# tnibler/local-features

Measured on AMD Instinct MI355X. Metric: MKD descriptors/sec (32x32 patch, 128-D), higher is better.
Workload: dtype f32 (f16x3 split MFMA pooling)

## Files before the change

local-features_amd/csrc/lf_mkd.cpp:

```cpp
#include "../../include/lf_mkd.h"

#include <hip/hip_runtime.h>

#include <algorithm>
#include <chrono>
#include <cmath>
#include <cstdlib>
#include <cstring>
#include <new>
#include <string>
#include <utility>
#include <vector>

#include "lf_mkd_internal.h"
#include "mkd_consts.hpp"
#include "mkd_device.h"

using namespace lfmkd;

namespace {

enum Memory { kDevice, kPinned };

template <typename T, Memory M = kDevice, bool Recorded = false>
// ... 107 lines not shown
struct DetectPlan {
    Recording graph;
    std::vector<uint32_t> cuts;
    std::vector<Recording> heads;
};

}

struct lf_mkd {
    lf_mkd_params params{};
    hipStream_t stream = nullptr;
    hipStream_t side_stream = nullptr;
    std::vector<hipEvent_t> side_events;
    struct {
        HipArray<short> colmap, colmap_unfolded;
        HipArray<float> pool_b_f32, white_a_f32, white_bias;
        HipArray<uint16_t> pool_b_f16, pool_b_fp6, white_a_f16, white_a_f16_unfolded;
    } consts;
    DeviceConsts dc;
    uint64_t batch = 0;
    HipArray<float> d_patches;
    HipArray<float> d_out;
    HipArray<float> d_kps;
    PyramidDesc pd{};
    HipArray<float> d_image, d_pyr, d_tmp_a, d_tmp_b;
    bool have_image = false;
    uint32_t max_frames = 1, n_frames = 0;
    long pyr_stride = 0;
    int n_layers = 7;
    HipArray<float> d_coarse;
    long layer_stride = 0, coarse_stride = 0;
// ... 158 lines not shown
        LF_CREATE_HIP(hipGetDeviceProperties(&prop, params->device));
        h->num_cus = prop.multiProcessorCount > 0 ? prop.multiProcessorCount : 256;
    }
    auto &c = h->consts;
    LF_CREATE_HIP(upload(c.colmap, hc.colmap));
    LF_CREATE_HIP(upload(c.pool_b_f32, hc.pool_b_f32));
    LF_CREATE_HIP(upload(c.pool_b_f16, hc.pool_b_f16));
    if (h->params.pool_mode == LF_MKD_POOL_F16_FP6) {
        LF_CREATE_HIP(upload(c.pool_b_fp6, hc.pool_b_fp6));
        LF_CREATE_HIP(upload(c.colmap_unfolded, hc.colmap_unfolded));
        LF_CREATE_HIP(upload(c.white_a_f16_unfolded, hc.white_a_f16_unfolded));
    }
    LF_CREATE_HIP(upload(c.white_a_f16, hc.white_a_f16));
    LF_CREATE_HIP(upload(c.white_a_f32, hc.white_a_f32));
    LF_CREATE_HIP(upload(c.white_bias, hc.white_bias));
    h->dc = DeviceConsts{c.colmap, c.pool_b_f32, c.pool_b_f16, c.white_a_f16, c.white_a_f32, c.colmap_unfolded, c.pool_b_fp6,
                         c.white_a_f16_unfolded, c.white_bias};
    LF_CREATE_HIP(h->d_totals.allocate(8));
    if (h->params.flags & LF_MKD_FLAG_KERNEL_TIMING) {
        LF_CREATE_HIP(h->d_clk.allocate(4));
        LF_CREATE_HIP(hipMemset(h->d_clk, 0, 4 * sizeof(unsigned long long)));
    }
    if (params->max_image_width && params->max_image_height) {
        if ((uint64_t(params->max_image_width) + 2 * kPyrApron) * (uint64_t(params->max_image_height) + 2 * kPyrApron) >= (1ull << 30) ||
            params->max_image_width >= (1u << 20) || params->max_image_height >= (1u << 20)) {
            h->err = "max_image_width x max_image_height (with the pyramid's apron of 48 texels a side) must stay below 2^30 pixels";
            return bail(LF_MKD_ERR_BAD_ARG);
        }
        h->max_frames = params->max_frames ? params->max_frames : 1;
        const size_t px = size_t(params->max_image_width) * params->max_image_height * h->max_frames;
        h->pyr_stride = pyramid_floats(params->max_image_width, params->max_image_height);
        h->layer_stride = long(params->max_image_width) * params->max_image_height;
// ... 334 lines not shown

int lfmkd_test_pool_tables(const float *mean, const float *eigvals, const float *eigvecs, float *pool_b_f32, int16_t *colmap, float *parity_defect) {
    if (!mean || !eigvals || !eigvecs) return LF_MKD_ERR_BAD_ARG;
    PcaModel pca;
    pca.mean.assign(mean, mean + kRaw);
    pca.eigvals.assign(eigvals, eigvals + kRaw);
    pca.eigvecs.assign(eigvecs, eigvecs + size_t(kRaw) * kRaw);
    HostConsts hc;
    if (const std::string e = build_host_consts(pca, hc); !e.empty()) {
        g_create_error = e;
        return LF_MKD_ERR_BAD_ARG;
    }
    if (pool_b_f32) std::memcpy(pool_b_f32, hc.pool_b_f32.data(), hc.pool_b_f32.size() * 4);
    if (colmap) std::memcpy(colmap, hc.colmap.data(), hc.colmap.size() * 2);
    if (parity_defect) *parity_defect = hc.lut_parity_defect;
    return LF_MKD_OK;
}

int lf_mkd_plan_upload(uint32_t width, uint32_t height, uint32_t bytes_per_pixel, uint32_t n_scales, uint32_t *cuts,
                       uint32_t max_cuts, uint32_t *n_cuts, double *modelled_us, double *one_piece_us) {
    if (!n_cuts || (bytes_per_pixel != 1 && bytes_per_pixel != 4) || width < 2 || height < 2 || (max_cuts && !cuts))
        return LF_MKD_ERR_BAD_ARG;
    const int n_layers = int(n_scales ? n_scales : 4) + 3;
    if (n_layers - 1 > 8) return LF_MKD_ERR_BAD_ARG;
    const std::vector<uint32_t> c = plan_cuts(n_layers, width, height, bytes_per_pixel == 1);
    *n_cuts = uint32_t(c.size());
    for (size_t i = 0; i < c.size() && i < max_cuts; ++i) cuts[i] = c[i];
    const FrontModel m;
    if (modelled_us) *modelled_us = front_finish_us(c, c.size() + 1, int(width), int(height), int(bytes_per_pixel), n_layers, m);
    if (one_piece_us) *one_piece_us = front_finish_us({}, 1, int(width), int(height), int(bytes_per_pixel), n_layers, m);
// ... 1154 lines not shown
```

local-features_amd/csrc/mkd_consts.cpp:

```cpp
#include "mkd_consts.hpp"

#include <cmath>
#include <cstdio>
#include <cstdlib>
#include <cstring>

namespace lfmkd {

namespace {

const float kVmN3K8[4] = {0.37872374f, 0.51796234f, 0.46882015f, 0.39798096f};
const float kVmN1K1[2] = {0.618176f, 0.6934725f};
const float kVmN2K8[3] = {0.37872374f, 0.51796234f, 0.46882015f};

struct Grid {
    float x[kPx], y[kPx];
    Grid() {
        for (int r = 0; r < kPatch; ++r)
            for (int c = 0; c < kPatch; ++c) {
                x[r * kPatch + c] = 2.f * float(c) / float(kPatch - 1) - 1.f;
                y[r * kPatch + c] = 2.f * float(r) / float(kPatch - 1) - 1.f;
            }
    }
};
// ... 248 lines not shown
        for (int y = 0; y < kPatch; ++y)
            for (int x = 0; x < kPatch / 2; ++x) {
                const double a = lut_value(col, y * kPatch + x), b = lut_value(col, y * kPatch + kPatch - 1 - x);
                even_err = std::fmax(even_err, std::fabs(a - b));
                odd_err = std::fmax(odd_err, std::fabs(a + b));
                mx = std::fmax(mx, std::fmax(std::fabs(a), std::fabs(b)));
            }
        defect = std::fmax(defect, float(std::fmin(even_err, odd_err) / mx));
        return memo = even_err <= odd_err ? 1 : -1;
    };
    FoldLayout fl;
    if (const std::string e = build_fold_layout(parity, fl); !e.empty()) return e;
    hc.lut_parity_defect = defect;
    if (!(defect < 1e-4f))
        return "internal: a pooling LUT column is neither even nor odd in x (defect " + std::to_string(defect) + ")";
    hc.colmap.assign(kPackedCols, -1);
    {
        std::vector<int> seen(kRaw, 0);
        for (int t = 0; t < kTiles; ++t) {
            int ut, v;
            acc_tile_source(t, ut, v);
            for (int c = 0; c < kTileCols; ++c) {
                const FoldColumn &fc = fl.col[ut][c];
                const int d = v ? fc.desc_v : fc.desc_u;
                if (d < 0) continue;
                hc.colmap[t * kTileCols + c] = int16_t(v && fc.sign_v < 0 ? -2 - d : d);
                ++seen[d];
            }
        }
        for (int d = 0; d < kRaw; ++d)
// ... 118 lines not shown
```

local-features_amd/csrc/mkd_consts.hpp:

```cpp
#pragma once
#include <cstdint>
#include <string>
#include <vector>

namespace lfmkd {

constexpr int kPatch = 32;
constexpr int kPx = kPatch * kPatch;
constexpr int kDimsIn = 7;
constexpr int kCart = 9;
constexpr int kPolar = 25;
constexpr int kRaw = 238;
constexpr int kOut = 128;

constexpr int kStreams = 7;
constexpr int kTiles = 21;
constexpr int kAccTiles = kTiles;
constexpr int kTileCols = 16;
constexpr int kPolarSlots = 10;
constexpr int kPackedCols = kTiles * kTileCols;
constexpr int kUniqueTiles = 12;

constexpr int kUnfAccTiles = 24;
constexpr int kUnfUniqueTiles = 15;
// ... 8 lines not shown
    std::vector<float> gradient_angle;
    std::vector<float> embedding_polar;
    std::vector<float> embedding_cartesian;
    std::vector<float> mean;
    std::vector<float> w_t;

    std::vector<int16_t> colmap;
    std::vector<float> pool_b_f32;
    std::vector<uint16_t> pool_b_f16;
    std::vector<uint16_t> white_a_f16;
    std::vector<float> white_a_f32;
    std::vector<int16_t> colmap_unfolded;
    std::vector<uint16_t> pool_b_fp6;
    std::vector<uint16_t> white_a_f16_unfolded;
    float lut_parity_defect = 0.f;
    std::vector<float> white_bias;
};

std::string build_host_consts(const PcaModel &pca, HostConsts &out);

}
```

local-features_amd/csrc/mkd_describe.hip:

```cpp
#include <hip/hip_runtime.h>
#include <stdint.h>

#include <type_traits>

#include "mkd_ablate.h"
#include "mkd_device.h"
#include "mkd_sample.h"

namespace lfmkd {


namespace {

typedef _Float16 f16x8 __attribute__((ext_vector_type(8)));
typedef unsigned int u32x4 __attribute__((ext_vector_type(4)));
typedef float f32x2 __attribute__((ext_vector_type(2)));
__device__ __forceinline__ f32x2 pk_fma(f32x2 a, f32x2 b, f32x2 c) { return __builtin_elementwise_fma(a, b, c); }
__device__ __forceinline__ f32x2 pk_set(float v) { return f32x2{v, v}; }

__device__ __host__ constexpr bool f16_family(int pool) { return pool == LF_POOL_F16X3 || pool == LF_POOL_F16_FP6; }

__device__ __host__ constexpr bool fold_form(int pool) { return pool != LF_POOL_F16_FP6; }
constexpr int kTiles = 21;
constexpr int kAccTiles = 21, kUnfAccTiles = 24;
__device__ __host__ constexpr int acc_tiles(bool fold) { return fold ? kAccTiles : kUnfAccTiles; }
__device__ __host__ constexpr int lut_pieces(bool fold) { return fold ? 24 : 30; }
constexpr int kPolarSlots = 10;

constexpr float kB0 = 0.0096f, kB1 = 0.2054f, kB2 = 0.5699f;

__device__ __host__ constexpr int row_bytes(bool fold) { return lut_pieces(fold) * 1024; }
__device__ __host__ constexpr int ring_off(bool fold) { return 2 * row_bytes(fold); }
constexpr int kRowBytes = row_bytes(true), kRingOff = ring_off(true);
constexpr int kRingSlots = 6;
[[maybe_unused]] constexpr int kSrcPatches = 0, kSrcKeypoints = 1, kSrcKeypointsSplit = 2;
constexpr int kRingSlotsKp = 12;
constexpr int kLevelTableBytes = 5 * kMaxPyrLevels * 4;

__device__ __forceinline__ float lane_fetch(int byte_addr, float v) {
    return __int_as_float(__builtin_amdgcn_ds_bpermute(byte_addr, __float_as_int(v)));
}

__device__ __forceinline__ void lds_dma16(const void *gsrc, void *ldst) {
    __builtin_amdgcn_global_load_lds((const __attribute__((address_space(1))) void *)gsrc,
                                     (__attribute__((address_space(3))) void *)ldst, 16, 0, 0);
}
__device__ __forceinline__ void lds_dma16_sv(const unsigned char *uniform_base, unsigned lane_off, void *ldst) {
    asm("" : "+s"(uniform_base));
    asm volatile("" : "+v"(lane_off));
    lds_dma16(uniform_base + lane_off, ldst);
}

template <int W, bool FOLD = true>
__device__ __forceinline__ void issue_lut_row(const unsigned char *__restrict__ lut_rows, int row,
                                              unsigned char *lds_row, int wave, int lane) {
    constexpr int kPieces = lut_pieces(FOLD);
    const unsigned lane16 = (unsigned)lane * 16u;
#pragma unroll
    for (int j = 0; j < (kPieces + W - 1) / W; ++j) {
        if (wave + W * j < kPieces) {
            const unsigned char *g = lut_rows + ((size_t)row * row_bytes(FOLD) + (size_t)(wave + W * j) * 1024);
            lds_dma16_sv(g, lane16, lds_row + (wave + W * j) * 1024);
        }
    }
}

constexpr int kWStepBytes = 16384;
__device__ __forceinline__ constexpr int wstage_slot(int step) { return step % 3 == 0 ? 0 : (step % 3 == 1 ? 32768 : 16384); }
static_assert(wstage_slot(0) + kWStepBytes <= row_bytes(true) && wstage_slot(10) >= row_bytes(false) &&
              wstage_slot(10) + kWStepBytes <= 2 * row_bytes(true), "both forms' row buffers");

template <int W>
__device__ __forceinline__ void issue_w_step(const unsigned char *__restrict__ wfrag, int step, unsigned char *lds,
                                             int wave, int lane) {
    const unsigned lane16 = (unsigned)lane * 16u;
    unsigned char *d = lds + wstage_slot(step);
#pragma unroll
// ... 340 lines not shown
    }
#pragma unroll
    for (int x = 0; x < 4; ++x) out[4 + x] = ob[3 - x];
    const float hal = lane_fetch(addr_l, out[3]), hbr = lane_fetch(addr_l, ob[0]);
    const float har = lane_fetch(addr_r, out[0]), hbl = lane_fetch(addr_r, ob[3]);
    nb[0] = has_l ? hal : out[0];
    nb[1] = has_r ? har : ob[0];
    nb[2] = has_r ? hbl : out[3];
    nb[3] = has_l ? hbr : ob[3];
}

__device__ __forceinline__ void fold_sum(const f32x2 (&s)[4], f32x2 &e0, f32x2 &e1) { e0 = s[0] + s[2]; e1 = s[1] + s[3]; }
__device__ __forceinline__ void fold_diff(const f32x2 (&s)[4], f32x2 &o0, f32x2 &o1) { o0 = s[0] - s[2]; o1 = s[1] - s[3]; }
__device__ __forceinline__ void fold_diff_rev(const f32x2 (&s)[4], f32x2 &o0, f32x2 &o1) { o0 = s[2] - s[0]; o1 = s[3] - s[1]; }

template <int POOL>
__device__ __forceinline__ void pool_harmonics(const f32x2 (&m)[4], const f32x2 (&c1)[4], const f32x2 (&s1)[4],
                                               const unsigned char *brow, BFrag &g, f32x4 (&acc)[kAccTiles]) {
    f32x2 pk[4], qk[4], pp[4], qp[4], tc[4];
    AFrag<POOL> au, av;
#pragma unroll
    for (int e = 0; e < 4; ++e) { pk[e] = m[e] * c1[e]; qk[e] = m[e] * s1[e]; tc[e] = c1[e] + c1[e]; }
#pragma unroll
    for (int k = 0; k < 3; ++k) {
        {
            f32x2 u[4], v[4];
            fold_sum(pk, u[0], u[1]);
            fold_diff(qk, u[2], u[3]);
            fold_sum(qk, v[0], v[1]);
            fold_diff_rev(pk, v[2], v[3]);
            if constexpr (POOL == LF_POOL_F16X3) {
                AFrag<POOL>::set2(au, u, av, v);
            } else {
                au.set(u);
                av.set(v);
            }
        }
        if (k < 2) {
#pragma unroll
            for (int e = 0; e < 4; ++e) {
                const f32x2 pn = pk_fma(tc[e], pk[e], k == 0 ? -m[e] : -pp[e]);
                const f32x2 qn = k == 0 ? tc[e] * qk[e] : pk_fma(tc[e], qk[e], -qp[e]);
                pp[e] = pk[e]; qp[e] = qk[e];
                pk[e] = pn; qk[e] = qn;
            }
        }
        const int a0 = 3 + 6 * k, u0 = 3 + 3 * k;
        const BFrag t0 = g, t1 = load_b(brow, u0 + 1), t2 = load_b(brow, u0 + 2);
        if (k < 2) g = load_b(brow, u0 + 3);
        mma_part<POOL, 0>(au, t0, acc[a0 + 0]); mma_part<POOL, 0>(av, t0, acc[a0 + 1]); mma_part<POOL, 0>(au, t1, acc[a0 + 2]);
        mma_part<POOL, 0>(av, t1, acc[a0 + 3]); mma_part<POOL, 0>(au, t2, acc[a0 + 4]); mma_part<POOL, 0>(av, t2, acc[a0 + 5]);
        mma_part<POOL, 1>(au, t0, acc[a0 + 0]); mma_part<POOL, 1>(av, t0, acc[a0 + 1]); mma_part<POOL, 1>(au, t1, acc[a0 + 2]);
        mma_part<POOL, 1>(av, t1, acc[a0 + 3]); mma_part<POOL, 1>(au, t2, acc[a0 + 4]); mma_part<POOL, 1>(av, t2, acc[a0 + 5]);
        mma_part<POOL, 2>(au, t0, acc[a0 + 0]); mma_part<POOL, 2>(av, t0, acc[a0 + 1]); mma_part<POOL, 2>(au, t1, acc[a0 + 2]);
        mma_part<POOL, 2>(av, t1, acc[a0 + 3]); mma_part<POOL, 2>(au, t2, acc[a0 + 4]); mma_part<POOL, 2>(av, t2, acc[a0 + 5]);
    }
}

typedef float v16f __attribute__((ext_vector_type(16)));
typedef unsigned v6u __attribute__((ext_vector_type(6)));
typedef int v8i __attribute__((ext_vector_type(8)));

__device__ __forceinline__ void pool_harmonics_fp6(const f32x2 (&m)[4], const f32x2 (&c1)[4], const f32x2 (&s1)[4],
// ... 188 lines not shown
#pragma unroll
            for (int rr = 0; rr < 4; ++rr)
                o[r0 + rr] = __builtin_amdgcn_mfma_f32_16x16x32_f16(__builtin_bit_cast(f16x8, src[2 * rr]), yl, o[r0 + rr], 0, 0, 0);
#pragma unroll
            for (int rr = 0; rr < 4; ++rr)
                o[r0 + rr] = __builtin_amdgcn_mfma_f32_16x16x32_f16(__builtin_bit_cast(f16x8, src[2 * rr]), yh, o[r0 + rr], 0, 0, 0);
        };
#pragma unroll
        for (int s = 0; s < 11; ++s) {
            if (s == 0) wait_vmcnt<2 * kDma>();
            else if (s < 10) wait_vmcnt<kDma>();
            else wait_vmcnt<0>();
            asm volatile("s_waitcnt lgkmcnt(0)" ::: "memory");
            __syncthreads();
            if (s >= 1 && s + 2 < 11) issue_w_step<W>(wfrag, s + 2, s_mem, wave, lane);
            if (s == 10 && more) issue_lut_row<W, kFold>(lut_rows, 0, s_mem, wave, lane);
            read_unit(2 * s, wbuf[0]);
            __builtin_amdgcn_sched_barrier(0);
            if (s > 0) mma_unit(2 * s - 1, wbuf[1]);
            {
                const f32x4 y0 = acc[2 * s];
                const f32x4 y1 = 2 * s + 1 < kTiles ? acc[(2 * s + 1 < kTiles) ? 2 * s + 1 : 0] : f32x4{0.f, 0.f, 0.f, 0.f};
                const f32x2 y[4] = {{y0[0], y0[1]}, {y0[2], y0[3]}, {y1[0], y1[1]}, {y1[2], y1[3]}};
                AFrag<LF_POOL_F16X3> yb;
                yb.set(y);
                yh = __builtin_bit_cast(f16x8, yb.hi);
                yl = __builtin_bit_cast(f16x8, yb.lo);
            }
            __builtin_amdgcn_sched_barrier(0);
            read_unit(2 * s + 1, wbuf[1]);
            __builtin_amdgcn_sched_barrier(0);
// ... 199 lines not shown
    sm.load_geometry(walk.cur, 0);
#pragma unroll 1
    for (int quarter = 0; quarter < 7; ++quarter) {
        sm.request(quarter, 0, ta);
        sm.finish(quarter, 0, 0, ta);
    }
    sm.request(7, 0, ta);
#pragma unroll 1
    for (long batch = walk.cur; batch < walk.end; batch += walk.step) {
        const bool more = batch + walk.step < walk.end;
        if (more) sm.load_geometry(batch + walk.step, set ^ 1);
        const int slot1 = (slot0 + 8) % kRingSlotsKp;
        auto step = [&](int g, KpTaps &cur, KpTaps &nxt) {
            asm volatile("s_waitcnt vmcnt(0) lgkmcnt(0)" ::: "memory");
            __syncthreads();
            if (g < 31) issue_lut_row<W>(lut_rows, g + 1, s_mem + ((g + 1) & 1) * kRowBytes, pw, lane);
            const int qn = g + 8;
            if (qn < 32) sm.request(qn, set, nxt);
            else if (more) sm.request(qn - 32, set ^ 1, nxt);
            __builtin_amdgcn_sched_barrier(0);
            const int qc = g + 7;
            if (qc < 32) sm.finish(qc, set, slot0, cur);
            else if (more) sm.finish(qc - 32, set ^ 1, slot1, cur);
        };
#pragma unroll 1
        for (int g = 0; g < ablate::kRows; g += 2) {
            step(g, ta, tb);
            step(g + 1, tb, ta);
        }
        asm volatile("s_waitcnt vmcnt(0) lgkmcnt(0)" ::: "memory");
#pragma unroll 1
// ... 29 lines not shown
    sm.load_geometry(batch, 0);
    sm.request(sp.q_first, 0, ta);
#pragma unroll 1
    for (int i = 0; i + 1 < sp.n_pro; i += 2) {
        sm.request(sp.q_first + i + 1, 0, tb);
        sm.finish(sp.q_first + i, 0, 0, ta);
        sm.request(sp.q_first + i + 2, 0, ta);
        sm.finish(sp.q_first + i + 1, 0, 0, tb);
    }
    sm.finish(sp.q_first + sp.n_pro - 1, 0, 0, ta);
    const int q_step0 = sp.q_first + sp.n_pro;
    if (q_step0 < sp.q_end) sm.request(q_step0, 0, ta);
    auto step = [&](int st, KpTaps &cur, KpTaps &nxt) {
        asm volatile("s_waitcnt vmcnt(0) lgkmcnt(0)" ::: "memory");
        __syncthreads();
        if (sp.lo + st + 1 < sp.hi) issue_lut_row<W>(lut_rows, sp.lo + st + 1, s_mem + ((st + 1) & 1) * kRowBytes, pw, lane);
        if (q_step0 + st + 1 < sp.q_end) sm.request(q_step0 + st + 1, 0, nxt);
        __builtin_amdgcn_sched_barrier(0);
        if (q_step0 + st < sp.q_end) sm.finish(q_step0 + st, 0, 0, cur);
    };
#pragma unroll 1
    for (int st = 0; st < sp.hi - sp.lo; st += 2) {
        step(st, ta, tb);
        step(st + 1, tb, ta);
    }
    asm volatile("s_waitcnt vmcnt(0) lgkmcnt(0)" ::: "memory");
    if (sp.consumer) {
#pragma unroll 1
        for (int e = 0; e < 12; ++e) __syncthreads();
    }
}

constexpr int kSplitSpinMax = 1 << 21;

}

template <int ANGLE, int POOL, int W, int SRC>
__global__ __launch_bounds__(SRC != kSrcPatches ? 128 * W : 64 * W) void mkd_pool(
    const float *__restrict__ patches, long n_host, const unsigned long long *__restrict__ n_dev,
    const unsigned char *__restrict__ lut_rows, const short *__restrict__ colmap, const unsigned char *__restrict__ wfrag,
    const float *__restrict__ bias, float *__restrict__ out, float *__restrict__ raw_out,
    std::conditional_t<SRC != kSrcPatches, KpSource, int> ks, unsigned long long *__restrict__ clk) {
    constexpr bool kKp = SRC != kSrcPatches, kSplit = SRC == kSrcKeypointsSplit;
    static_assert(!kSplit || W == 2, "the row-split form is the narrow (2 + 2 wave) form");
    if (clk && blockIdx.x == 0 && threadIdx.x == 0) {
        clk[0] = __builtin_readcyclecounter();
        clk[1] = __builtin_amdgcn_s_memrealtime();
    }
    constexpr int kSlots = kKp ? kRingSlotsKp : kRingSlots;
    static_assert(!kKp || POOL == LF_POOL_F16X3, "keypoint mode pools in f16x3");
    constexpr int kMPool = POOL == LF_POOL_F16_FP6 ? LF_POOL_F16X3 : POOL;
    constexpr bool kFold = fold_form(POOL);
    static_assert(!kKp || kFold, "the producers write the folded forms' LDS map");
    constexpr int kNAcc = acc_tiles(kFold), kRowB = row_bytes(kFold), kRingO = ring_off(kFold);
    __shared__ __attribute__((aligned(16))) unsigned char s_mem[kRingO + W * kSlots * 2048 +
                                                                (kKp ? kLevelTableBytes + kMaxPyrLevels * 8 : 0)];
    const long n = n_dev ? (long)*n_dev : n_host;
    const int lane = threadIdx.x & 63;
    const int wave = __builtin_amdgcn_readfirstlane(threadIdx.x >> 6);
    const int p = lane & 15, q = lane >> 4;
    const int addr_l = ((lane - 16) & 63) * 4, addr_r = ((lane + 16) & 63) * 4;
    const bool has_l = q > 0, has_r = q < 3;
    const long nbatch = (n + 16 * W - 1) / (16 * W);
    unsigned char *ring = s_mem + kRingO + wave * (kSlots * 2048);
    BatchWalk walk{(long)blockIdx.x, nbatch, (long)gridDim.x};
    [[maybe_unused]] RowSpan span{0, 32, 0, 32, 7, true};
    [[maybe_unused]] int role = 0, n_roles = 1;
    if constexpr (kKp) {
// ... 23 lines not shown
        __syncthreads();
        const LevelTable lt{ks.pd.levels, lv, lv + kMaxPyrLevels, lv + 2 * kMaxPyrLevels, lv + 3 * kMaxPyrLevels};
        if (wave >= W) {
            if constexpr (kSplit) kp_produce_split<W>(ks, lt, lv_off, n, walk.cur, span, s_mem, lut_rows, wave - W, lane);
            else kp_produce<W>(ks, lt, lv_off, n, walk, s_mem, lut_rows, wave - W, lane);
            return;
        }

        if constexpr (ablate::kConsumerPrio >= 0) __builtin_amdgcn_s_setprio(ablate::kConsumerPrio);
    }
    const unsigned char *ring_lane = kFold ? ring + (q * 16 + p) * 16 : ring + (q >> 1) * 1024 + ((2 * (q & 1)) * 16 + p) * 16;
    [[maybe_unused]] const unsigned char *ring_mirror = ring + 1024 + ((3 - q) * 16 + p) * 16;

    long batch = walk.cur;
    if (batch >= walk.end) return;
    auto raw_src = [&](const float *pt, long b) {
        const long b0 = b * (16 * W) + wave * 16;
        const long wave0 = b0 < n ? b0 : n - 1;
        const long pidx = b0 + p < n ? b0 + p : n - 1;
        return RawSrc{reinterpret_cast<const unsigned char *>(pt + wave0 * 1024), (unsigned)(pidx - wave0) * 4096u + 16u * q};
    };
    {
        if constexpr (!kKp) {
            const RawSrc src = raw_src(patches, batch);
#pragma unroll
            for (int r = -2; r <= 3; ++r) issue_raw_row(src, r, ring, r + 2);
        }
        issue_lut_row<W, kFold>(lut_rows, kSplit ? span.lo : 0, s_mem, wave, lane);
    }
    int slot0 = 0;
    unsigned par = 0;
    ablate::PhaseClock phase;
    phase.start();

    for (; batch < walk.end; batch += walk.step) {
        const unsigned char *wf = wfrag, *lr = lut_rows;
        const float *bs = bias, *pt = patches;
        float *o = out, *ro = raw_out;
        const short *cm = colmap;
        asm volatile("" : "+s"(wf), "+s"(bs), "+s"(lr), "+s"(o), "+s"(ro), "+s"(cm), "+s"(pt));
        const long base = batch * (16 * W) + wave * 16;
        const bool more = batch + walk.step < walk.end;
        const RawSrc src = kKp ? RawSrc{nullptr, 0u} : raw_src(pt, batch);
        const RawSrc src_next = !kKp && more ? raw_src(pt, batch + walk.step) : src;

        f32x4 acc[kNAcc];
#pragma unroll
        for (int t = 0; t < kNAcc; ++t) acc[t] = f32x4{0.f, 0.f, 0.f, 0.f};
        float cur[8], prv[8], cur_nb[4] = {0.f, 0.f, 0.f, 0.f};
        int s0 = 1;

        auto patch_row = [&](auto kind, const int g) __attribute__((always_inline)) {
            constexpr bool kFirst = decltype(kind)::value == 0, kLast = decltype(kind)::value == 2;
            constexpr bool kFirstInner = decltype(kind)::value == 3;

            phase.mark(7);
            if constexpr (!ablate::kNoRowSync) {
                asm volatile("s_waitcnt vmcnt(0)" ::: "memory");
                __syncthreads();
            }
            phase.mark(0);
            const unsigned char *brow = s_mem + par * kRowB + lane * 16;
            if (f16_family(POOL) ? !kLast : (!kLast || more)) {
                if constexpr (!kKp) issue_lut_row<W, kFold>(lr, (g + 1) & 31, s_mem + (par ^ 1) * kRowB, wave, lane);
            } else if (f16_family(POOL)) {
                issue_w_step<W>(wf, 0, s_mem, wave, lane);
            }
            par ^= 1;
            BFrag bm[3] = {load_b(brow, 0), load_b(brow, 1), load_b(brow, 2)};

            if constexpr (!kKp)
                if (!kFirst && !kLast && g <= 29) issue_raw_row(src, g + 4, ring, s0 == 0 ? kRingSlots - 1 : s0 - 1);
            auto kp_slot = [&](int y, int i) {
                int r_ = y - 2 + i;
                r_ = r_ < 0 ? 0 : (r_ > 31 ? 31 : r_);
                return (slot0 + r_) % kRingSlotsKp;
            };
            auto blur = [&](auto tap, float (&o)[8], float (&o_nb)[4]) __attribute__((always_inline)) {
                if constexpr (kFold) blur_row_fold_impl(ring_lane, ring_mirror, tap, addr_l, addr_r, has_l, has_r, o, o_nb);
                else blur_row_impl(ring_lane, tap, addr_l, addr_r, has_l, has_r, o, o_nb[0], o_nb[1]);
            };
            auto ring_tap = [](int first) {
                return [first](int i) { const int sl = first + i; return sl >= kRingSlots ? sl - kRingSlots : sl; };
            };
// ... 64 lines not shown
            for (int x = 0; x < 8; ++x) {
                prv[x] = cur[x];
                cur[x] = nxt[x];
            }
#pragma unroll
            for (int x = 0; x < 4; ++x) cur_nb[x] = nxt_nb[x];
            phase.mark(2);

            BFrag gfrag = load_b(brow, 3);
            {
                AFrag<kMPool> am;
                if constexpr (kFold) {
                    f32x2 mf[4];
                    fold_sum(m, mf[0], mf[1]);
                    fold_diff(m, mf[2], mf[3]);
                    am.set(mf);
                } else {
                    am.set(m);
                }
#pragma unroll
                for (int t = 0; t < 3; ++t) mma_part<kMPool, 0>(am, bm[t], acc[t]);
#pragma unroll
                for (int t = 0; t < 3; ++t) mma_part<kMPool, 1>(am, bm[t], acc[t]);
#pragma unroll
                for (int t = 0; t < 3; ++t) mma_part<kMPool, 2>(am, bm[t], acc[t]);
            }
            phase.mark(3);
            if constexpr (POOL == LF_POOL_F16_FP6) pool_harmonics_fp6(m, c1, s1, brow, gfrag, acc);
            else pool_harmonics<POOL>(m, c1, s1, brow, gfrag, acc);
            phase.mark(4);
            phase.mark(5);
        };
        if constexpr (kSplit) {
            if (span.lo == 0) patch_row(std::integral_constant<int, 0>(), 0);
            else patch_row(std::integral_constant<int, 3>(), span.lo);
#pragma unroll 1
            for (int g = span.lo + 1; g < span.hi - 1; ++g) patch_row(std::integral_constant<int, 1>(), g);
            if (span.consumer) patch_row(std::integral_constant<int, 2>(), span.hi - 1);
            else patch_row(std::integral_constant<int, 1>(), span.hi - 1);
            unsigned *cnt = ks.xchg_cnt + batch * W + wave;
            typedef unsigned long long u64;
            if (!span.consumer) {
                u64 *dst = reinterpret_cast<u64 *>(ks.xchg + ((((long)batch * (n_roles - 1) + role) * W + wave) * kAccTiles) * 256) + lane;
#pragma unroll
                for (int t = 0; t < kAccTiles; ++t) {
                    const u64 v0 = ((u64)__float_as_uint(acc[t][1]) << 32) | __float_as_uint(acc[t][0]);
                    const u64 v1 = ((u64)__float_as_uint(acc[t][3]) << 32) | __float_as_uint(acc[t][2]);
                    __hip_atomic_store(dst + t * 128, v0, __ATOMIC_RELAXED, __HIP_MEMORY_SCOPE_AGENT);
                    __hip_atomic_store(dst + t * 128 + 64, v1, __ATOMIC_RELAXED, __HIP_MEMORY_SCOPE_AGENT);
                }
                asm volatile("s_waitcnt vmcnt(0)" ::: "memory");
                if (lane == 0) __hip_atomic_fetch_add(cnt, 1u, __ATOMIC_RELAXED, __HIP_MEMORY_SCOPE_AGENT);
                if (clk && blockIdx.x == 0 && threadIdx.x == 0) {
                    clk[2] = __builtin_readcyclecounter();
// ... 17 lines not shown
                for (int t = 0; t < 2 * kAccTiles; ++t)
                    v[t] = __hip_atomic_load(srcp + t * 64, __ATOMIC_RELAXED, __HIP_MEMORY_SCOPE_AGENT);
                __builtin_amdgcn_sched_barrier(0);
#pragma unroll
                for (int t = 0; t < kAccTiles; ++t)
                    acc[t] += f32x4{__uint_as_float((unsigned)v[2 * t]), __uint_as_float((unsigned)(v[2 * t] >> 32)),
                                    __uint_as_float((unsigned)v[2 * t + 1]), __uint_as_float((unsigned)(v[2 * t + 1] >> 32))};
            }
            if (lane == 0) __hip_atomic_store(cnt, 0u, __ATOMIC_RELAXED, __HIP_MEMORY_SCOPE_AGENT);
            asm volatile("s_waitcnt vmcnt(0)" ::: "memory");
        } else {
            patch_row(std::integral_constant<int, 0>(), 0);
#pragma unroll 1
            for (int g = 1; g < ablate::kRows - 1; ++g) patch_row(std::integral_constant<int, 1>(), g);
            patch_row(std::integral_constant<int, 2>(), ablate::kRows - 1);
        }
        if constexpr (ablate::kNoEpilogue) {
            f32x4 sum = acc[0];
            for (int t = 1; t < kNAcc; ++t) sum += acc[t];
            if (base + p < n) *reinterpret_cast<f32x4 *>(out + (base + p) * 128 + 4 * q) = sum;
            if (f16_family(POOL)) {
                __syncthreads();
                if (more) issue_lut_row<W, kFold>(lr, 0, s_mem, wave, lane);
            }
        } else {
            finish_descriptors<POOL, W>(acc, lane, wave, base + p < n, base + p, cm, wf, bs, o, ro, s_mem, lr, more);
        }
        phase.mark(6);
        if constexpr (kKp) slot0 = (slot0 + 8) % kRingSlotsKp;
    }
    phase.dump(out, wave, lane);
    if (clk && blockIdx.x == 0 && threadIdx.x == 0) {
        clk[2] = __builtin_readcyclecounter();
        clk[3] = __builtin_amdgcn_s_memrealtime();
    }
}

#ifndef LF_DESCRIBE_KP
// ... 3 lines not shown
    if (n <= 0) return;
    const bool small = ablate::kForceFourWaves || waves == 4 || (waves != 8 && n <= 64L * num_cus);
    const long nbatch = small ? (n + 63) / 64 : (n + 127) / 128;
    const unsigned grid = (unsigned)(nbatch < num_cus ? nbatch : num_cus);
    const bool f16 = f16_family(pool_mode);
    const unsigned char *lut = pool_mode == LF_POOL_F16_FP6 ? reinterpret_cast<const unsigned char *>(dc.pool_b_fp6)
                               : f16                        ? reinterpret_cast<const unsigned char *>(dc.pool_b_f16)
                                                            : reinterpret_cast<const unsigned char *>(dc.pool_b_f32);
    const bool unfolded = !fold_form(pool_mode);
    const unsigned char *wf = unfolded ? reinterpret_cast<const unsigned char *>(dc.white_a_f16_unfolded)
                              : f16    ? reinterpret_cast<const unsigned char *>(dc.white_a_f16)
                                       : reinterpret_cast<const unsigned char *>(dc.white_a_f32);
    const short *colmap = unfolded ? dc.colmap_unfolded : dc.colmap;
#define LF_LAUNCH_W(A, P, WV)                                                                                          \
    hipLaunchKernelGGL((mkd_pool<A, P, WV, kSrcPatches>), dim3(grid), dim3(64 * WV), 0, stream, patches, n, n_dev, lut, \
                       colmap, wf, dc.white_bias, out, raw_out, 0, clk)
#define LF_LAUNCH(A, P)            \
    do {                           \
        if (small) LF_LAUNCH_W(A, P, 4); \
        else LF_LAUNCH_W(A, P, 8); \
    } while (0)
    if (pool_mode == LF_POOL_F16_FP6) {
        if (angle_mode == LF_ANGLE_EXACT) LF_LAUNCH(LF_ANGLE_EXACT, LF_POOL_F16_FP6);
        else if (angle_mode == LF_ANGLE_EXACT_ZERO) LF_LAUNCH(LF_ANGLE_EXACT_ZERO, LF_POOL_F16_FP6);
        else LF_LAUNCH(LF_ANGLE_SHADER, LF_POOL_F16_FP6);
    } else if (f16) {
        if (angle_mode == LF_ANGLE_EXACT) LF_LAUNCH(LF_ANGLE_EXACT, LF_POOL_F16X3);
        else if (angle_mode == LF_ANGLE_EXACT_ZERO) LF_LAUNCH(LF_ANGLE_EXACT_ZERO, LF_POOL_F16X3);
        else LF_LAUNCH(LF_ANGLE_SHADER, LF_POOL_F16X3);
    } else {
        if (angle_mode == LF_ANGLE_EXACT) LF_LAUNCH(LF_ANGLE_EXACT, LF_POOL_F32);
// ... 27 lines not shown
    ks.pyr = pyr; ks.pyr_stride = pyr_stride; ks.kps = kps; ks.frame_of = frame_of_kp; ks.n_frames = n_frames ? n_frames : 1u;
    ks.psf = psf; ks.pd = pd;
    ks.split = 1; ks.xchg = nullptr; ks.xchg_cnt = nullptr;
    if (xchg && xchg_words) {
        const long nf8 = (nbatch32(form_n) + 7) / 8 * 8, nb8 = (nbatch32(n) + 7) / 8 * 8;
        int r = nf8 * 4 <= num_cus ? 4 : (nf8 * 2 <= num_cus ? 2 : 1);
        if (const char *e = getenv("LF_MKD_KP_SPLIT")) {
            const int want = atoi(e);
            if (want == 1 || ((want == 2 || want == 4) && nf8 * want <= num_cus)) r = want;
        }
        if (r > 1) {
            ks.split = r; ks.xchg = xchg; ks.xchg_cnt = xchg_words + 1;
            const unsigned sgrid = (unsigned)(nb8 * r);
#define LF_LAUNCH_KP_SPLIT(A)                                                                                                  \
    hipLaunchKernelGGL((mkd_pool<A, LF_POOL_F16X3, 2, kSrcKeypointsSplit>), dim3(sgrid), dim3(256), 0, stream,                    \
                       (const float *)nullptr, n, n_dev, lut, dc.colmap, wf, dc.white_bias, out, (float *)nullptr, ks, clk)
            if (angle_mode == LF_ANGLE_EXACT) LF_LAUNCH_KP_SPLIT(LF_ANGLE_EXACT);
            else if (angle_mode == LF_ANGLE_EXACT_ZERO) LF_LAUNCH_KP_SPLIT(LF_ANGLE_EXACT_ZERO);
            else LF_LAUNCH_KP_SPLIT(LF_ANGLE_SHADER);
#undef LF_LAUNCH_KP_SPLIT
            return;
        }
    }
#define LF_LAUNCH_KP_W(A, WV)                                                                                          \
    hipLaunchKernelGGL((mkd_pool<A, LF_POOL_F16X3, WV, kSrcKeypoints>), dim3(grid), dim3(128 * WV), 0, stream,          \
                       (const float *)nullptr, n, n_dev, lut, dc.colmap, wf, dc.white_bias, out, (float *)nullptr, ks, clk)
#define LF_LAUNCH_KP(A)                 \
    do {                                \
        if (narrow) LF_LAUNCH_KP_W(A, 2); \
        else LF_LAUNCH_KP_W(A, 4);      \
    } while (0)
    if (angle_mode == LF_ANGLE_EXACT) LF_LAUNCH_KP(LF_ANGLE_EXACT);
    else if (angle_mode == LF_ANGLE_EXACT_ZERO) LF_LAUNCH_KP(LF_ANGLE_EXACT_ZERO);
    else LF_LAUNCH_KP(LF_ANGLE_SHADER);
#undef LF_LAUNCH_KP_W
#undef LF_LAUNCH_KP
}
#endif

}
```

local-features_amd/csrc/mkd_device.h:

```cpp
#pragma once
#include <hip/hip_runtime.h>

#include <functional>
#include <stdint.h>

#include "mkd_verify_pair.h"

#define LF_ANGLE_SHADER 0
#define LF_ANGLE_EXACT 1
#define LF_ANGLE_EXACT_ZERO 2
#define LF_POOL_F16X3 1
#define LF_POOL_F32 2
#define LF_POOL_F16_FP6 3

namespace lfmkd {

typedef float f32x4 __attribute__((ext_vector_type(4)));

constexpr int kMaxPyrLevels = 16;

constexpr int kPyrApron = 48;
struct PyramidDesc {
    int levels;
    int w[kMaxPyrLevels], h[kMaxPyrLevels];
// ... 8 lines not shown
    int layer_lo[8], layer_hi[8];
    int scan_lo, scan_hi;
};
bool plan_row_bands(int raw_rows, int w, int h, int n_layers, int border, RowBands &bands);

struct DeviceConsts {
    short *colmap = nullptr;
    float *pool_b_f32 = nullptr;
    uint16_t *pool_b_f16 = nullptr;
    uint16_t *white_a_f16 = nullptr;
    float *white_a_f32 = nullptr;
    short *colmap_unfolded = nullptr;
    uint16_t *pool_b_fp6 = nullptr;
    uint16_t *white_a_f16_unfolded = nullptr;
    float *white_bias = nullptr;
};

void launch_describe(const float *patches, long n, const unsigned long long *n_dev, const DeviceConsts &dc,
                     int angle_mode, int pool_mode, float *out, float *raw_out, int num_cus, hipStream_t stream,
                     int waves = 0, unsigned long long *clk = nullptr);
void launch_sample_patches(const float *pyr, long pyr_stride, const PyramidDesc &pd, const float *kps,
                           const unsigned *frame_of_kp, unsigned n_frames, long n, const unsigned long long *n_dev, float psf,
                           float *patches, hipStream_t stream);
void launch_describe_keypoints(const float *pyr, long pyr_stride, const PyramidDesc &pd, const float *kps,
                               const unsigned *frame_of_kp, unsigned n_frames, long n, const unsigned long long *n_dev,
                               float psf, const DeviceConsts &dc, int angle_mode, float *out, int num_cus, hipStream_t stream,
                               unsigned long long *clk = nullptr, float *xchg = nullptr, unsigned *xchg_words = nullptr,
                               long form_n = 0);
size_t kp_split_exchange_bytes(int num_cus);
size_t kp_split_counter_words(int num_cus);
// ... 92 lines not shown
```

Measured before the change: 294.5 million.

## Pool x-odd cartesian kernels as separable VALU sums instead of MFMA tiles

```diff
diff --git a/local-features_amd/csrc/lf_mkd.cpp b/local-features_amd/csrc/lf_mkd.cpp
--- a/local-features_amd/csrc/lf_mkd.cpp
+++ b/local-features_amd/csrc/lf_mkd.cpp
@@ -145,7 +145,7 @@
     std::vector<hipEvent_t> side_events;
     struct {
         HipArray<short> colmap, colmap_unfolded;
-        HipArray<float> pool_b_f32, white_a_f32, white_bias;
+        HipArray<float> pool_b_f32, white_a_f32, white_bias, odd_cart;
         HipArray<uint16_t> pool_b_f16, pool_b_fp6, white_a_f16, white_a_f16_unfolded;
     } consts;
     DeviceConsts dc;
@@ -334,8 +334,13 @@
     LF_CREATE_HIP(upload(c.white_a_f16, hc.white_a_f16));
     LF_CREATE_HIP(upload(c.white_a_f32, hc.white_a_f32));
     LF_CREATE_HIP(upload(c.white_bias, hc.white_bias));
+    {
+        std::vector<float> oc(hc.odd_cart_fx, hc.odd_cart_fx + 16);
+        oc.insert(oc.end(), &hc.odd_cart_gy[0][0], &hc.odd_cart_gy[0][0] + 32 * 4);
+        LF_CREATE_HIP(upload(c.odd_cart, oc));
+    }
     h->dc = DeviceConsts{c.colmap, c.pool_b_f32, c.pool_b_f16, c.white_a_f16, c.white_a_f32, c.colmap_unfolded, c.pool_b_fp6,
-                         c.white_a_f16_unfolded, c.white_bias};
+                         c.white_a_f16_unfolded, c.white_bias, c.odd_cart};
     LF_CREATE_HIP(h->d_totals.allocate(8));
     if (h->params.flags & LF_MKD_FLAG_KERNEL_TIMING) {
         LF_CREATE_HIP(h->d_clk.allocate(4));
@@ -700,6 +705,23 @@
     if (pool_b_f32) std::memcpy(pool_b_f32, hc.pool_b_f32.data(), hc.pool_b_f32.size() * 4);
     if (colmap) std::memcpy(colmap, hc.colmap.data(), hc.colmap.size() * 2);
     if (parity_defect) *parity_defect = hc.lut_parity_defect;
+    return LF_MKD_OK;
+}
+
+int lfmkd_test_pool_factors(const float *mean, const float *eigvals, const float *eigvecs, float *fx, float *gy, float *defect) {
+    if (!mean || !eigvals || !eigvecs) return LF_MKD_ERR_BAD_ARG;
+    PcaModel pca;
+    pca.mean.assign(mean, mean + kRaw);
+    pca.eigvals.assign(eigvals, eigvals + kRaw);
+    pca.eigvecs.assign(eigvecs, eigvecs + size_t(kRaw) * kRaw);
+    HostConsts hc;
+    if (const std::string e = build_host_consts(pca, hc); !e.empty()) {
+        g_create_error = e;
+        return LF_MKD_ERR_BAD_ARG;
+    }
+    if (fx) std::memcpy(fx, hc.odd_cart_fx, sizeof hc.odd_cart_fx);
+    if (gy) std::memcpy(gy, hc.odd_cart_gy, sizeof hc.odd_cart_gy);
+    if (defect) *defect = hc.odd_cart_defect;
     return LF_MKD_OK;
 }
 
diff --git a/local-features_amd/csrc/mkd_consts.cpp b/local-features_amd/csrc/mkd_consts.cpp
--- a/local-features_amd/csrc/mkd_consts.cpp
+++ b/local-features_amd/csrc/mkd_consts.cpp
@@ -286,6 +286,44 @@
     hc.lut_parity_defect = defect;
     if (!(defect < 1e-4f))
         return "internal: a pooling LUT column is neither even nor odd in x (defect " + std::to_string(defect) + ")";
+    {
+        for (int k = 0; k <= 3; ++k)
+            for (int i = 0; i < kCart; ++i)
+                if ((parity(LutColumn{true, false, i, k, 0}) < 0) != (i >= 6))
+                    return "internal: the x-odd cartesian kernels are not EC 6, 7, 8";
+        const double half_pi = 3.14159265358979323846 / 2.0, mn2 = double(max_norm) * double(max_norm);
+        auto vm1 = [&](int a, double t) {
+            return a == 0 ? double(kVmN1K1[0]) : (a == 1 ? std::cos(t) : std::sin(t)) * double(kVmN1K1[1]);
+        };
+        auto fx = [&](int x) {
+            const double g = grid.x[x];
+            return vm1(2, g * half_pi) * std::exp(-(g * g) / mn2);
+        };
+        for (int x = 0; x < kPatch / 2; ++x) hc.odd_cart_fx[x] = float(0.5 * (fx(x) - fx(kPatch - 1 - x)));
+        for (int y = 0; y < kPatch; ++y) {
+            const double g = grid.y[y * kPatch];
+            for (int b = 0; b < 3; ++b) hc.odd_cart_gy[y][b] = float(vm1(b, g * half_pi) * std::exp(-(g * g) / mn2));
+            hc.odd_cart_gy[y][3] = 0.f;
+        }
+        double worst = 0.0;
+        for (int k = 0; k <= 3; ++k)
+            for (int b = 0; b < 3; ++b) {
+                const LutColumn col{true, false, 6 + b, k, 0};
+                double err = 0.0, mx = 0.0;
+                for (int y = 0; y < kPatch; ++y)
+                    for (int x = 0; x < kPatch; ++x) {
+                        const double f = x < kPatch / 2 ? hc.odd_cart_fx[x] : -double(hc.odd_cart_fx[kPatch - 1 - x]);
+                        const double v = lut_value_d(col, y * kPatch + x);
+                        err = std::fmax(err, std::fabs(double(kVmN3K8[k]) * f * double(hc.odd_cart_gy[y][b]) - v));
+                        mx = std::fmax(mx, std::fabs(v));
+                    }
+                worst = std::fmax(worst, err / mx);
+            }
+        hc.odd_cart_defect = float(worst);
+        if (!(hc.odd_cart_defect < 1e-6f))
+            return "internal: the x-odd cartesian kernels are not a product of an x- and a y-profile (defect " +
+                   std::to_string(hc.odd_cart_defect) + ")";
+    }
     hc.colmap.assign(kPackedCols, -1);
     {
         std::vector<int> seen(kRaw, 0);
diff --git a/local-features_amd/csrc/mkd_consts.hpp b/local-features_amd/csrc/mkd_consts.hpp
--- a/local-features_amd/csrc/mkd_consts.hpp
+++ b/local-features_amd/csrc/mkd_consts.hpp
@@ -46,6 +46,9 @@
     std::vector<uint16_t> pool_b_fp6;
     std::vector<uint16_t> white_a_f16_unfolded;
     float lut_parity_defect = 0.f;
+    float odd_cart_fx[16] = {};
+    float odd_cart_gy[32][4] = {};
+    float odd_cart_defect = 0.f;
     std::vector<float> white_bias;
 };
 
diff --git a/local-features_amd/csrc/mkd_describe.hip b/local-features_amd/csrc/mkd_describe.hip
--- a/local-features_amd/csrc/mkd_describe.hip
+++ b/local-features_amd/csrc/mkd_describe.hip
@@ -25,6 +25,8 @@
 constexpr int kAccTiles = 21, kUnfAccTiles = 24;
 __device__ __host__ constexpr int acc_tiles(bool fold) { return fold ? kAccTiles : kUnfAccTiles; }
 __device__ __host__ constexpr int lut_pieces(bool fold) { return fold ? 24 : 30; }
+__device__ __host__ constexpr bool valu_odd_cart(int pool) { return pool == LF_POOL_F16X3; }
+constexpr int kOddCartSums = 7;
 constexpr int kPolarSlots = 10;
 
 constexpr float kB0 = 0.0096f, kB1 = 0.2054f, kB2 = 0.5699f;
@@ -51,16 +53,18 @@
     lds_dma16(uniform_base + lane_off, ldst);
 }
 
-template <int W, bool FOLD = true>
+template <int W, bool FOLD, bool ODDV>
 __device__ __forceinline__ void issue_lut_row(const unsigned char *__restrict__ lut_rows, int row,
                                               unsigned char *lds_row, int wave, int lane) {
-    constexpr int kPieces = lut_pieces(FOLD);
+    static_assert(!ODDV || FOLD, "the folded forms' tiles");
+    constexpr int kPieces = ODDV ? lut_pieces(FOLD) - 8 : lut_pieces(FOLD);
     const unsigned lane16 = (unsigned)lane * 16u;
 #pragma unroll
     for (int j = 0; j < (kPieces + W - 1) / W; ++j) {
         if (wave + W * j < kPieces) {
-            const unsigned char *g = lut_rows + ((size_t)row * row_bytes(FOLD) + (size_t)(wave + W * j) * 1024);
-            lds_dma16_sv(g, lane16, lds_row + (wave + W * j) * 1024);
+            const int i = wave + W * j, piece = ODDV ? i + 2 * (i >> 2) : i;
+            const unsigned char *g = lut_rows + ((size_t)row * row_bytes(FOLD) + (size_t)piece * 1024);
+            lds_dma16_sv(g, lane16, lds_row + piece * 1024);
         }
     }
 }
@@ -431,9 +435,30 @@
 __device__ __forceinline__ void fold_diff(const f32x2 (&s)[4], f32x2 &o0, f32x2 &o1) { o0 = s[0] - s[2]; o1 = s[1] - s[3]; }
 __device__ __forceinline__ void fold_diff_rev(const f32x2 (&s)[4], f32x2 &o0, f32x2 &o1) { o0 = s[2] - s[0]; o1 = s[3] - s[1]; }
 
+__device__ __forceinline__ void odd_cart_row(const f32x2 (&fx)[2], const f32x4 &gy, f32x2 h0, f32x2 h1, float (&oc)[3]) {
+    const f32x2 r = pk_fma(fx[1], h1, fx[0] * h0);
+    const float t = r.x + r.y;
+#pragma unroll
+    for (int b = 0; b < 3; ++b) oc[b] = __builtin_fmaf(gy[b], t, oc[b]);
+}
+
+__device__ __forceinline__ void rebuild_odd_cart(const float (&oc)[kOddCartSums][3], int lane, f32x4 (&acc)[kAccTiles]) {
+    constexpr float kVm[4] = {0.37872374f, 0.51796234f, 0.46882015f, 0.39798096f};
+#pragma unroll
+    for (int s = 0; s < kOddCartSums; ++s) {
+        const int k = (s + 1) / 2, t = s == 0 ? 2 : 3 + 6 * (k - 1) + 4 + ((s - 1) & 1);
+        f32x4 d = {0.f, 0.f, 0.f, 0.f};
+#pragma unroll
+        for (int b = 0; b < 3; ++b)
+            d = __builtin_amdgcn_mfma_f32_16x16x4f32((lane & 15) == b ? kVm[k] : 0.f, oc[s][b], d, 0, 0, 0);
+        acc[t] = d;
+    }
+}
+
 template <int POOL>
 __device__ __forceinline__ void pool_harmonics(const f32x2 (&m)[4], const f32x2 (&c1)[4], const f32x2 (&s1)[4],
-                                               const unsigned char *brow, BFrag &g, f32x4 (&acc)[kAccTiles]) {
+                                               const unsigned char *brow, BFrag &g, f32x4 (&acc)[kAccTiles],
+                                               const f32x2 (&fx)[2], const f32x4 &gy, float (&oc)[kOddCartSums][3]) {
     f32x2 pk[4], qk[4], pp[4], qp[4], tc[4];
     AFrag<POOL> au, av;
 #pragma unroll
@@ -446,6 +471,10 @@
             fold_diff(qk, u[2], u[3]);
             fold_sum(qk, v[0], v[1]);
             fold_diff_rev(pk, v[2], v[3]);
+            if constexpr (valu_odd_cart(POOL)) {
+                odd_cart_row(fx, gy, u[2], u[3], oc[1 + 2 * k]);
+                odd_cart_row(fx, gy, v[2], v[3], oc[2 + 2 * k]);
+            }
             if constexpr (POOL == LF_POOL_F16X3) {
                 AFrag<POOL>::set2(au, u, av, v);
             } else {
@@ -463,7 +492,18 @@
             }
         }
         const int a0 = 3 + 6 * k, u0 = 3 + 3 * k;
-        const BFrag t0 = g, t1 = load_b(brow, u0 + 1), t2 = load_b(brow, u0 + 2);
+        const BFrag t0 = g, t1 = load_b(brow, u0 + 1);
+        if constexpr (valu_odd_cart(POOL)) {
+            if (k < 2) g = load_b(brow, u0 + 3);
+            mma_part<POOL, 0>(au, t0, acc[a0 + 0]); mma_part<POOL, 0>(av, t0, acc[a0 + 1]); mma_part<POOL, 0>(au, t1, acc[a0 + 2]);
+            mma_part<POOL, 0>(av, t1, acc[a0 + 3]);
+            mma_part<POOL, 1>(au, t0, acc[a0 + 0]); mma_part<POOL, 1>(av, t0, acc[a0 + 1]); mma_part<POOL, 1>(au, t1, acc[a0 + 2]);
+            mma_part<POOL, 1>(av, t1, acc[a0 + 3]);
+            mma_part<POOL, 2>(au, t0, acc[a0 + 0]); mma_part<POOL, 2>(av, t0, acc[a0 + 1]); mma_part<POOL, 2>(au, t1, acc[a0 + 2]);
+            mma_part<POOL, 2>(av, t1, acc[a0 + 3]);
+            continue;
+        }
+        const BFrag t2 = load_b(brow, u0 + 2);
         if (k < 2) g = load_b(brow, u0 + 3);
         mma_part<POOL, 0>(au, t0, acc[a0 + 0]); mma_part<POOL, 0>(av, t0, acc[a0 + 1]); mma_part<POOL, 0>(au, t1, acc[a0 + 2]);
         mma_part<POOL, 0>(av, t1, acc[a0 + 3]); mma_part<POOL, 0>(au, t2, acc[a0 + 4]); mma_part<POOL, 0>(av, t2, acc[a0 + 5]);
@@ -682,7 +722,7 @@
             asm volatile("s_waitcnt lgkmcnt(0)" ::: "memory");
             __syncthreads();
             if (s >= 1 && s + 2 < 11) issue_w_step<W>(wfrag, s + 2, s_mem, wave, lane);
-            if (s == 10 && more) issue_lut_row<W, kFold>(lut_rows, 0, s_mem, wave, lane);
+            if (s == 10 && more) issue_lut_row<W, kFold, valu_odd_cart(POOL)>(lut_rows, 0, s_mem, wave, lane);
             read_unit(2 * s, wbuf[0]);
             __builtin_amdgcn_sched_barrier(0);
             if (s > 0) mma_unit(2 * s - 1, wbuf[1]);
@@ -912,7 +952,7 @@
         auto step = [&](int g, KpTaps &cur, KpTaps &nxt) {
             asm volatile("s_waitcnt vmcnt(0) lgkmcnt(0)" ::: "memory");
             __syncthreads();
-            if (g < 31) issue_lut_row<W>(lut_rows, g + 1, s_mem + ((g + 1) & 1) * kRowBytes, pw, lane);
+            if (g < 31) issue_lut_row<W, true, true>(lut_rows, g + 1, s_mem + ((g + 1) & 1) * kRowBytes, pw, lane);
             const int qn = g + 8;
             if (qn < 32) sm.request(qn, set, nxt);
             else if (more) sm.request(qn - 32, set ^ 1, nxt);
@@ -972,7 +1012,7 @@
     auto step = [&](int st, KpTaps &cur, KpTaps &nxt) {
         asm volatile("s_waitcnt vmcnt(0) lgkmcnt(0)" ::: "memory");
         __syncthreads();
-        if (sp.lo + st + 1 < sp.hi) issue_lut_row<W>(lut_rows, sp.lo + st + 1, s_mem + ((st + 1) & 1) * kRowBytes, pw, lane);
+        if (sp.lo + st + 1 < sp.hi) issue_lut_row<W, true, true>(lut_rows, sp.lo + st + 1, s_mem + ((st + 1) & 1) * kRowBytes, pw, lane);
         if (q_step0 + st + 1 < sp.q_end) sm.request(q_step0 + st + 1, 0, nxt);
         __builtin_amdgcn_sched_barrier(0);
         if (q_step0 + st < sp.q_end) sm.finish(q_step0 + st, 0, 0, cur);
@@ -997,7 +1037,7 @@
 __global__ __launch_bounds__(SRC != kSrcPatches ? 128 * W : 64 * W) void mkd_pool(
     const float *__restrict__ patches, long n_host, const unsigned long long *__restrict__ n_dev,
     const unsigned char *__restrict__ lut_rows, const short *__restrict__ colmap, const unsigned char *__restrict__ wfrag,
-    const float *__restrict__ bias, float *__restrict__ out, float *__restrict__ raw_out,
+    const float *__restrict__ bias, const float *__restrict__ odd_cart, float *__restrict__ out, float *__restrict__ raw_out,
     std::conditional_t<SRC != kSrcPatches, KpSource, int> ks, unsigned long long *__restrict__ clk) {
     constexpr bool kKp = SRC != kSrcPatches, kSplit = SRC == kSrcKeypointsSplit;
     static_assert(!kSplit || W == 2, "the row-split form is the narrow (2 + 2 wave) form");
@@ -1008,8 +1048,8 @@
     constexpr int kSlots = kKp ? kRingSlotsKp : kRingSlots;
     static_assert(!kKp || POOL == LF_POOL_F16X3, "keypoint mode pools in f16x3");
     constexpr int kMPool = POOL == LF_POOL_F16_FP6 ? LF_POOL_F16X3 : POOL;
-    constexpr bool kFold = fold_form(POOL);
-    static_assert(!kKp || kFold, "the producers write the folded forms' LDS map");
+    constexpr bool kFold = fold_form(POOL), kOddV = valu_odd_cart(POOL);
+    static_assert(!kKp || (kFold && kOddV), "the producers write the folded forms' LDS map and request f16x3's LUT pieces");
     constexpr int kNAcc = acc_tiles(kFold), kRowB = row_bytes(kFold), kRingO = ring_off(kFold);
     __shared__ __attribute__((aligned(16))) unsigned char s_mem[kRingO + W * kSlots * 2048 +
                                                                 (kKp ? kLevelTableBytes + kMaxPyrLevels * 8 : 0)];
@@ -1063,6 +1103,13 @@
 
     long batch = walk.cur;
     if (batch >= walk.end) return;
+    [[maybe_unused]] f32x2 oc_fx[2] = {pk_set(0.f), pk_set(0.f)};
+    if constexpr (kOddV) {
+        const f32x4 f = *reinterpret_cast<const f32x4 *>(odd_cart + 4 * q);
+        oc_fx[0] = f32x2{f[0], f[1]};
+        oc_fx[1] = f32x2{f[2], f[3]};
+        asm volatile("" : "+v"(oc_fx[0]), "+v"(oc_fx[1]));
+    }
     auto raw_src = [&](const float *pt, long b) {
         const long b0 = b * (16 * W) + wave * 16;
         const long wave0 = b0 < n ? b0 : n - 1;
@@ -1075,7 +1122,7 @@
 #pragma unroll
             for (int r = -2; r <= 3; ++r) issue_raw_row(src, r, ring, r + 2);
         }
-        issue_lut_row<W, kFold>(lut_rows, kSplit ? span.lo : 0, s_mem, wave, lane);
+        issue_lut_row<W, kFold, kOddV>(lut_rows, kSplit ? span.lo : 0, s_mem, wave, lane);
     }
     int slot0 = 0;
     unsigned par = 0;
@@ -1088,6 +1135,7 @@
         float *o = out, *ro = raw_out;
         const short *cm = colmap;
         asm volatile("" : "+s"(wf), "+s"(bs), "+s"(lr), "+s"(o), "+s"(ro), "+s"(cm), "+s"(pt));
+        const float *oc_tab = odd_cart;
         const long base = batch * (16 * W) + wave * 16;
         const bool more = batch + walk.step < walk.end;
         const RawSrc src = kKp ? RawSrc{nullptr, 0u} : raw_src(pt, batch);
@@ -1096,6 +1144,11 @@
         f32x4 acc[kNAcc];
 #pragma unroll
         for (int t = 0; t < kNAcc; ++t) acc[t] = f32x4{0.f, 0.f, 0.f, 0.f};
+        [[maybe_unused]] float oc[kOddCartSums][3];
+#pragma unroll
+        for (int s = 0; s < kOddCartSums; ++s)
+#pragma unroll
+            for (int b = 0; b < 3; ++b) oc[s][b] = 0.f;
         float cur[8], prv[8], cur_nb[4] = {0.f, 0.f, 0.f, 0.f};
         int s0 = 1;
 
@@ -1111,12 +1164,17 @@
             phase.mark(0);
             const unsigned char *brow = s_mem + par * kRowB + lane * 16;
             if (f16_family(POOL) ? !kLast : (!kLast || more)) {
-                if constexpr (!kKp) issue_lut_row<W, kFold>(lr, (g + 1) & 31, s_mem + (par ^ 1) * kRowB, wave, lane);
+                if constexpr (!kKp) issue_lut_row<W, kFold, kOddV>(lr, (g + 1) & 31, s_mem + (par ^ 1) * kRowB, wave, lane);
             } else if (f16_family(POOL)) {
                 issue_w_step<W>(wf, 0, s_mem, wave, lane);
             }
             par ^= 1;
-            BFrag bm[3] = {load_b(brow, 0), load_b(brow, 1), load_b(brow, 2)};
+            constexpr int kMTiles = kOddV ? 2 : 3;
+            BFrag bm[kMTiles];
+#pragma unroll
+            for (int t = 0; t < kMTiles; ++t) bm[t] = load_b(brow, t);
+            [[maybe_unused]] f32x4 oc_gy = {0.f, 0.f, 0.f, 0.f};
+            if constexpr (kOddV) oc_gy = *reinterpret_cast<const f32x4 *>(oc_tab + 16 + 4 * g);
 
             if constexpr (!kKp)
                 if (!kFirst && !kLast && g <= 29) issue_raw_row(src, g + 4, ring, s0 == 0 ? kRingSlots - 1 : s0 - 1);
@@ -1211,20 +1269,21 @@
                     f32x2 mf[4];
                     fold_sum(m, mf[0], mf[1]);
                     fold_diff(m, mf[2], mf[3]);
+                    if constexpr (kOddV) odd_cart_row(oc_fx, oc_gy, mf[2], mf[3], oc[0]);
                     am.set(mf);
                 } else {
                     am.set(m);
                 }
 #pragma unroll
-                for (int t = 0; t < 3; ++t) mma_part<kMPool, 0>(am, bm[t], acc[t]);
-#pragma unroll
-                for (int t = 0; t < 3; ++t) mma_part<kMPool, 1>(am, bm[t], acc[t]);
-#pragma unroll
-                for (int t = 0; t < 3; ++t) mma_part<kMPool, 2>(am, bm[t], acc[t]);
+                for (int t = 0; t < kMTiles; ++t) mma_part<kMPool, 0>(am, bm[t], acc[t]);
+#pragma unroll
+                for (int t = 0; t < kMTiles; ++t) mma_part<kMPool, 1>(am, bm[t], acc[t]);
+#pragma unroll
+                for (int t = 0; t < kMTiles; ++t) mma_part<kMPool, 2>(am, bm[t], acc[t]);
             }
             phase.mark(3);
             if constexpr (POOL == LF_POOL_F16_FP6) pool_harmonics_fp6(m, c1, s1, brow, gfrag, acc);
-            else pool_harmonics<POOL>(m, c1, s1, brow, gfrag, acc);
+            else pool_harmonics<POOL>(m, c1, s1, brow, gfrag, acc, oc_fx, oc_gy, oc);
             phase.mark(4);
             phase.mark(5);
         };
@@ -1235,6 +1294,7 @@
             for (int g = span.lo + 1; g < span.hi - 1; ++g) patch_row(std::integral_constant<int, 1>(), g);
             if (span.consumer) patch_row(std::integral_constant<int, 2>(), span.hi - 1);
             else patch_row(std::integral_constant<int, 1>(), span.hi - 1);
+            if constexpr (kOddV) rebuild_odd_cart(oc, lane, acc);
             unsigned *cnt = ks.xchg_cnt + batch * W + wave;
             typedef unsigned long long u64;
             if (!span.consumer) {
@@ -1282,6 +1342,7 @@
 #pragma unroll 1
             for (int g = 1; g < ablate::kRows - 1; ++g) patch_row(std::integral_constant<int, 1>(), g);
             patch_row(std::integral_constant<int, 2>(), ablate::kRows - 1);
+            if constexpr (kOddV) rebuild_odd_cart(oc, lane, acc);
         }
         if constexpr (ablate::kNoEpilogue) {
             f32x4 sum = acc[0];
@@ -1289,7 +1350,7 @@
             if (base + p < n) *reinterpret_cast<f32x4 *>(out + (base + p) * 128 + 4 * q) = sum;
             if (f16_family(POOL)) {
                 __syncthreads();
-                if (more) issue_lut_row<W, kFold>(lr, 0, s_mem, wave, lane);
+                if (more) issue_lut_row<W, kFold, kOddV>(lr, 0, s_mem, wave, lane);
             }
         } else {
             finish_descriptors<POOL, W>(acc, lane, wave, base + p < n, base + p, cm, wf, bs, o, ro, s_mem, lr, more);
@@ -1323,7 +1384,7 @@
     const short *colmap = unfolded ? dc.colmap_unfolded : dc.colmap;
 #define LF_LAUNCH_W(A, P, WV)                                                                                          \
     hipLaunchKernelGGL((mkd_pool<A, P, WV, kSrcPatches>), dim3(grid), dim3(64 * WV), 0, stream, patches, n, n_dev, lut, \
-                       colmap, wf, dc.white_bias, out, raw_out, 0, clk)
+                       colmap, wf, dc.white_bias, dc.odd_cart, out, raw_out, 0, clk)
 #define LF_LAUNCH(A, P)            \
     do {                           \
         if (small) LF_LAUNCH_W(A, P, 4); \
@@ -1381,7 +1442,7 @@
             const unsigned sgrid = (unsigned)(nb8 * r);
 #define LF_LAUNCH_KP_SPLIT(A)                                                                                                  \
     hipLaunchKernelGGL((mkd_pool<A, LF_POOL_F16X3, 2, kSrcKeypointsSplit>), dim3(sgrid), dim3(256), 0, stream,                    \
-                       (const float *)nullptr, n, n_dev, lut, dc.colmap, wf, dc.white_bias, out, (float *)nullptr, ks, clk)
+                       (const float *)nullptr, n, n_dev, lut, dc.colmap, wf, dc.white_bias, dc.odd_cart, out, (float *)nullptr, ks, clk)
             if (angle_mode == LF_ANGLE_EXACT) LF_LAUNCH_KP_SPLIT(LF_ANGLE_EXACT);
             else if (angle_mode == LF_ANGLE_EXACT_ZERO) LF_LAUNCH_KP_SPLIT(LF_ANGLE_EXACT_ZERO);
             else LF_LAUNCH_KP_SPLIT(LF_ANGLE_SHADER);
@@ -1391,7 +1452,7 @@
     }
 #define LF_LAUNCH_KP_W(A, WV)                                                                                          \
     hipLaunchKernelGGL((mkd_pool<A, LF_POOL_F16X3, WV, kSrcKeypoints>), dim3(grid), dim3(128 * WV), 0, stream,          \
-                       (const float *)nullptr, n, n_dev, lut, dc.colmap, wf, dc.white_bias, out, (float *)nullptr, ks, clk)
+                       (const float *)nullptr, n, n_dev, lut, dc.colmap, wf, dc.white_bias, dc.odd_cart, out, (float *)nullptr, ks, clk)
 #define LF_LAUNCH_KP(A)                 \
     do {                                \
         if (narrow) LF_LAUNCH_KP_W(A, 2); \
diff --git a/local-features_amd/csrc/mkd_device.h b/local-features_amd/csrc/mkd_device.h
--- a/local-features_amd/csrc/mkd_device.h
+++ b/local-features_amd/csrc/mkd_device.h
@@ -46,6 +46,7 @@
     uint16_t *pool_b_fp6 = nullptr;
     uint16_t *white_a_f16_unfolded = nullptr;
     float *white_bias = nullptr;
+    float *odd_cart = nullptr;
 };
 
 void launch_describe(const float *patches, long n, const unsigned long long *n_dev, const DeviceConsts &dc,
```

New measurement: 307.0 million (median of 6 runs). 1.04x the previous value.
